# nghiant03/spine-vision

Measured on NVIDIA B200. Metric: series/sec, higher is better.
Workload: dtype fp16

## Files before the change

spine_vision_b200/csrc/svb_convnext_kernels.cuh:

```cuda
#pragma once
#include "svb_common.cuh"

namespace svb {

constexpr float LN_EPS_BACKBONE = 1e-6f;
constexpr float LN_EPS_HEAD = 1e-5f;
constexpr int DW_KX_UNROLL = 1;

__device__ __forceinline__ float gelu_fast(float x) {
    const float u = fminf(fabsf(x), 5.65685425f);
    float r = -5.20460508e-04f;
    r = fmaf(r, u, 7.39751849e-03f);
    r = fmaf(r, u, -5.25612477e-02f);
    r = fmaf(r, u, -4.59254682e-01f);
    r = fmaf(r, u, -1.15109138e+00f);
    r *= u;
    float e;
    asm("ex2.approx.ftz.f32 %0, %1;" : "=f"(e) : "f"(r));
    const float h = (0.5f * x) * e;
    return fmaxf(x, 0.0f) - fabsf(h);
}
__device__ __forceinline__ float gelu_exact(float x) { return 0.5f * x * (1.0f + erff(x * 0.70710678118654752f)); }

constexpr int STEM_TPW = 4;
// ... 871 lines not shown
                uint32_t r[32];
                tmem_ld_32x32(tmem_base + ((uint32_t)(q * 32) << 16) + (uint32_t)(as * BN + slice * CW + c * 32), r);
                if (MODE == GEMM_RESID) {
                    if (c > 0 && lane == 0) {
                        bulk_wait_read<0>();
                        mbar_expect_tx(rf, Cfg::EPI_BUF_BYTES);
                        tma_load_2d(ebuf_p, &resid_map, rf, col, row0);
                    }
                } else {
                    if (lane == 0) bulk_wait_read<0>();
                    __syncwarp();
                }
                tmem_ld_wait();
                if (MODE == GEMM_RESID) {
                    mbar_wait(rf, rph);
                    rph ^= 1u;
                }
#pragma unroll
                for (int i = 0; i < 4; ++i) {
                    const uint32_t addr = row_off + ((((uint32_t)i) ^ swz) << 4);
                    const float4 b0 = __ldg(reinterpret_cast<const float4*>(bias + col) + 2 * i);
                    const float4 b1 = __ldg(reinterpret_cast<const float4*>(bias + col) + 2 * i + 1);
                    uint64_t v01, v23, v45, v67;
                    if (MODE == GEMM_LNGELU) {
                        const float4 s0 = __ldg(reinterpret_cast<const float4*>(gamma + col) + 2 * i);
                        const float4 s1 = __ldg(reinterpret_cast<const float4*>(gamma + col) + 2 * i + 1);
                        v01 = fma2(ra2, pk2(__uint_as_float(r[8 * i + 0]), __uint_as_float(r[8 * i + 1])), fma2(rb2, pk2(s0.x, s0.y), pk2(b0.x, b0.y)));
                        v23 = fma2(ra2, pk2(__uint_as_float(r[8 * i + 2]), __uint_as_float(r[8 * i + 3])), fma2(rb2, pk2(s0.z, s0.w), pk2(b0.z, b0.w)));
                        v45 = fma2(ra2, pk2(__uint_as_float(r[8 * i + 4]), __uint_as_float(r[8 * i + 5])), fma2(rb2, pk2(s1.x, s1.y), pk2(b1.x, b1.y)));
                        v67 = fma2(ra2, pk2(__uint_as_float(r[8 * i + 6]), __uint_as_float(r[8 * i + 7])), fma2(rb2, pk2(s1.z, s1.w), pk2(b1.z, b1.w)));
                    } else {
                        v01 = add2(pk2(__uint_as_float(r[8 * i + 0]), __uint_as_float(r[8 * i + 1])), pk2(b0.x, b0.y));
                        v23 = add2(pk2(__uint_as_float(r[8 * i + 2]), __uint_as_float(r[8 * i + 3])), pk2(b0.z, b0.w));
                        v45 = add2(pk2(__uint_as_float(r[8 * i + 4]), __uint_as_float(r[8 * i + 5])), pk2(b1.x, b1.y));
                        v67 = add2(pk2(__uint_as_float(r[8 * i + 6]), __uint_as_float(r[8 * i + 7])), pk2(b1.z, b1.w));
                    }
                    uint4 o;
                    if (MODE == GEMM_GELU || MODE == GEMM_LNGELU) {
                        o = make_uint4(gelu_pack2<T>(v01), gelu_pack2<T>(v23), gelu_pack2<T>(v45), gelu_pack2<T>(v67));
                    } else {
                        if (MODE == GEMM_RESID) {
                            const float4 g0 = __ldg(reinterpret_cast<const float4*>(gamma + col) + 2 * i);
                            const float4 g1 = __ldg(reinterpret_cast<const float4*>(gamma + col) + 2 * i + 1);
                            const uint4 rv = lds128(addr);
                            const float2 x01 = Cvt<T>::unpack2(rv.x), x23 = Cvt<T>::unpack2(rv.y);
                            const float2 x45 = Cvt<T>::unpack2(rv.z), x67 = Cvt<T>::unpack2(rv.w);
                            v01 = fma2(pk2(g0.x, g0.y), v01, pk2(x01.x, x01.y));
                            v23 = fma2(pk2(g0.z, g0.w), v23, pk2(x23.x, x23.y));
                            v45 = fma2(pk2(g1.x, g1.y), v45, pk2(x45.x, x45.y));
                            v67 = fma2(pk2(g1.z, g1.w), v67, pk2(x67.x, x67.y));
                        }
                        float f0, f1, f2, f3, f4, f5, f6, f7;
                        upk2(v01, f0, f1); upk2(v23, f2, f3); upk2(v45, f4, f5); upk2(v67, f6, f7);
                        o = make_uint4(Cvt<T>::pack2(f0, f1), Cvt<T>::pack2(f2, f3), Cvt<T>::pack2(f4, f5), Cvt<T>::pack2(f6, f7));
                    }
                    sts128(addr, o);
                }
                fence_proxy_async();
                __syncwarp();
                if (lane == 0) {
                    tma_store_2d(&out_map, ebuf_p, col, row0);
                    bulk_commit();
                }
            }
            tc_fence_before();
            __syncwarp();
            if (lane == 0) {
                if (CG == 1 || rank == 0) mbar_arrive_relaxed(&tempty[as]);
                else mbar_arrive_cluster_relaxed(mapa_shared(smem_u32(&tempty[as]), 0));
            }
            if (++as == 2) { as = 0; aphase ^= 1; }
        }
        if (lane == 0) bulk_wait_all();
    }
    tc_fence_before();
    if (CG == 2) cluster_sync_all(); else __syncthreads();
    if (warp == 1) tmem_dealloc<CG>(tmem_base, Cfg::TMEM_COLS);
}

template <int C>
struct MlpCfg {
    static constexpr int HC = 64;
    static constexpr int NJ = 4 * C / HC;
    static constexpr int NB = (512 - C) / HC;
    static constexpr int KB_A = C / 64;
    static constexpr int A_BYTES = KB_A * 16384;
    static constexpr int H_BYTES = 16384;
    static constexpr int W1_KB_BYTES = 32 * 128;
    static constexpr int SLOT = KB_A * W1_KB_BYTES;
    static constexpr int W_SLOTS = C == 128 ? 7 : 5;
    static constexpr int VEC_BYTES = (4 * C + 4 * C + C + C) * 4;
    static constexpr int EPI_WARPS = 16;
    static constexpr int CH = C / 4 / 32;
    static constexpr bool STAGE_IN_H = C == 256;
    static constexpr int STAGE_BYTES = STAGE_IN_H ? 0 : EPI_WARPS * CH * 2048;
    static constexpr int NUM_THREADS = 64 + 32 * EPI_WARPS;
    static constexpr int NUM_BARS = 2 * W_SLOTS + 2 + 6 * NB + 4 + EPI_WARPS;
    static constexpr int SMEM_BYTES = A_BYTES + NB * H_BYTES + STAGE_BYTES + W_SLOTS * SLOT + VEC_BYTES + NUM_BARS * 8 + 64 + 1024;
    static constexpr int TMEM_COLS = 512;
    static_assert(C == 128 || C == 256, "Y (C columns) + NB 64-column hidden accumulators must fit 512 TMEM columns");
    static_assert(C + NB * HC <= 512, "TMEM budget");
    static_assert(SLOT == (C / 2) * 128, "W1 and W2 chunk halves are the same size");
    static_assert(!STAGE_IN_H || NB * H_BYTES >= EPI_WARPS * CH * 2048, "staging must fit the hidden buffers");
    static_assert(SMEM_BYTES <= 227 * 1024, "shared memory budget");
};

template <typename T, int C, bool LNF>
__global__ void __launch_bounds__(MlpCfg<C>::NUM_THREADS, 1)
mlp_fused_kernel(const __grid_constant__ CUtensorMap a_map, const __grid_constant__ CUtensorMap w1_map,
                 const __grid_constant__ CUtensorMap w2_map, const __grid_constant__ CUtensorMap x_map,
                 const float* __restrict__ b1, const float* __restrict__ b2, const float* __restrict__ gamma, int M,
                 const float* __restrict__ s1, const float2* __restrict__ rowstat, int stat_parts) {
    using Cfg = MlpCfg<C>;
    constexpr int NJ = Cfg::NJ, S = Cfg::W_SLOTS, NB = Cfg::NB, CH = Cfg::CH;
    extern __shared__ uint8_t smem_raw[];
    uint8_t* smem = smem_raw + ((1024u - (smem_u32(smem_raw) & 1023u)) & 1023u);
    uint8_t* sA = smem;
    uint8_t* sH = sA + Cfg::A_BYTES;
    uint8_t* sStage = sH + NB * Cfg::H_BYTES;
    uint8_t* sW = sStage + Cfg::STAGE_BYTES;
    float* sB1 = reinterpret_cast<float*>(sW + S * Cfg::SLOT);
    float* sS1 = sB1 + 4 * C;
    float* sB2 = sS1 + 4 * C;
    float* sGm = sB2 + C;
    uint64_t* bars = reinterpret_cast<uint64_t*>(reinterpret_cast<uint8_t*>(sB1) + Cfg::VEC_BYTES);
    uint64_t* wfull = bars;
    uint64_t* wempty = wfull + S;
    uint64_t* afull = wempty + S;
    uint64_t* aempty = afull + 1;
    uint64_t* hacc_full = aempty + 1;
    uint64_t* hacc_free_l = hacc_full + NB;
    uint64_t* hacc_free_p = hacc_free_l + NB;
    uint64_t* hs_full_l = hacc_free_p + NB;
    uint64_t* hs_full_p = hs_full_l + NB;
    uint64_t* hs_free = hs_full_p + NB;
    uint64_t* yfull = hs_free + NB;
    uint64_t* yfree_l = yfull + 1;
    uint64_t* yfree_p = yfree_l + 1;
    uint64_t* rfull = yfree_p + 2;
    uint32_t* tmem_ptr = reinterpret_cast<uint32_t*>(rfull + Cfg::EPI_WARPS);

    const int warp = __shfl_sync(0xffffffffu, (int)(threadIdx.x >> 5), 0), lane = threadIdx.x & 31;
    const uint32_t rank = cluster_ctarank();
    const int num_tiles = (M + 255) / 256;
    const int tile0 = (int)blockIdx.x / 2, tile_step = (int)gridDim.x / 2;

    if (warp == 0 && lane == 0) {
        tma_prefetch_desc(&a_map);
        tma_prefetch_desc(&w1_map);
        tma_prefetch_desc(&w2_map);
        tma_prefetch_desc(&x_map);
        for (int s = 0; s < S; ++s) { mbar_init(&wfull[s], 1); mbar_init(&wempty[s], 1); }
        mbar_init(afull, 1);
        mbar_init(aempty, 1);
        for (int s = 0; s < NB; ++s) {
            mbar_init(&hacc_full[s], 1);
            mbar_init(&hacc_free_l[s], Cfg::EPI_WARPS);
            mbar_init(&hacc_free_p[s], 1);
            mbar_init(&hs_full_l[s], Cfg::EPI_WARPS);
            mbar_init(&hs_full_p[s], 1);
            mbar_init(&hs_free[s], 1);
        }
        mbar_init(yfull, 1);
        mbar_init(yfree_l, Cfg::EPI_WARPS);
        mbar_init(yfree_p, 1);
        for (int s = 0; s < Cfg::EPI_WARPS; ++s) mbar_init(&rfull[s], 1);
        mbar_fence_init();
    }
    if (warp == 1) tmem_alloc<2>(tmem_ptr, Cfg::TMEM_COLS);
    for (int i = threadIdx.x; i < 4 * C; i += Cfg::NUM_THREADS) {
        sB1[i] = __ldg(b1 + i);
        sS1[i] = LNF ? __ldg(s1 + i) : 0.f;
    }
    for (int i = threadIdx.x; i < C; i += Cfg::NUM_THREADS) {
        sB2[i] = __ldg(b2 + i);
        sGm[i] = __ldg(gamma + i);
    }
    tc_fence_before();
    cluster_sync_all();
    tc_fence_after();
    const uint32_t tmem_base = *tmem_ptr;
    const uint32_t tm_y = tmem_base, tm_h = tmem_base + (uint32_t)C;
    pdl_launch_dependents();

    if (warp == 0) {
        if (lane == 0) {
            pdl_wait();
            int slot = 0;
            uint32_t wphase = 0, tcount = 0;
            auto next_slot = [&]() -> uint8_t* {
                mbar_wait(&wempty[slot], wphase ^ 1);
                if (rank == 0) mbar_expect_tx(&wfull[slot], 2 * Cfg::SLOT);
                return sW + slot * Cfg::SLOT;
            };
            auto advance = [&]() { if (++slot == S) { slot = 0; wphase ^= 1; } };
            auto load_w1 = [&](int j) {
                uint8_t* dst = next_slot();
                const uint32_t lb = mapa_shared(smem_u32(&wfull[slot]), 0);
#pragma unroll
                for (int kb = 0; kb < Cfg::KB_A; ++kb)
                    tma_load_2d_pair(dst + kb * Cfg::W1_KB_BYTES, &w1_map, lb, kb * 64, j * 64 + (int)rank * 32);
                advance();
            };
            auto load_w2 = [&](int jj) {
                uint8_t* dst = next_slot();
                const uint32_t lb = mapa_shared(smem_u32(&wfull[slot]), 0);
                tma_load_2d_pair(dst, &w2_map, lb, jj * 64, (int)rank * (C / 2));
                advance();
            };
            for (int tile = tile0; tile < num_tiles; tile += tile_step, ++tcount) {
                const int row_a = (tile * 2 + (int)rank) * 128;
                mbar_wait(aempty, (tcount & 1) ^ 1);
                if (rank == 0) mbar_expect_tx(afull, 2 * Cfg::A_BYTES);
                const uint32_t la = mapa_shared(smem_u32(afull), 0);
#pragma unroll
                for (int kb = 0; kb < Cfg::KB_A; ++kb) tma_load_2d_pair(sA + kb * 16384, &a_map, la, kb * 64, row_a);
                for (int j = 0; j < NJ + NB - 1; ++j) {
                    if (j < NJ) load_w1(j);
                    if (j >= NB - 1) load_w2(j - (NB - 1));
                }
            }
        }
    } else if (warp == 1) {
        if (rank == 0) {
            const uint32_t lead = elect_one() ? 1u : 0u;
            constexpr uint32_t idesc1 = (1u << 4) | (UmmaFmt<T>::v << 7) | (UmmaFmt<T>::v << 10) | ((uint32_t)(Cfg::HC >> 3) << 17) |
                                        ((uint32_t)(256 >> 4) << 24);
            constexpr uint32_t idesc2 = (1u << 4) | (UmmaFmt<T>::v << 7) | (UmmaFmt<T>::v << 10) | ((uint32_t)(C >> 3) << 17) |
                                        ((uint32_t)(256 >> 4) << 24);
            int slot = 0;
            uint32_t wphase = 0, tcount = 0, j1 = 0, j2 = 0;
            auto wait_slot = [&]() -> uint32_t {
                mbar_wait(&wfull[slot], wphase);
                tc_fence_after();
                return smem_u32(sW + slot * Cfg::SLOT);
            };
            auto release_slot = [&]() {
                tc_commit_if<2>(lead, &wempty[slot]);
                if (++slot == S) { slot = 0; wphase ^= 1; }
            };
            for (int tile = tile0; tile < num_tiles; tile += tile_step, ++tcount) {
                mbar_wait(afull, tcount & 1);
                tc_fence_after();
                for (int j = 0; j < NJ + NB - 1; ++j) {
                    if (j < NJ) {
                        const uint32_t hb = j1 % NB, par = ((j1 / NB) & 1) ^ 1;
                        mbar_wait(&hacc_free_l[hb], par);
                        mbar_wait(&hacc_free_p[hb], par);
                        tc_fence_after();
                        const uint32_t d = tm_h + hb * Cfg::HC;
                        {
                            const uint32_t wb = wait_slot();
#pragma unroll
                            for (int kb = 0; kb < Cfg::KB_A; ++kb) {
                                const uint64_t adesc = make_sw128_kmajor_desc(smem_u32(sA + kb * 16384));
                                const uint64_t bdesc = make_sw128_kmajor_desc(wb + kb * Cfg::W1_KB_BYTES);
#pragma unroll
                                for (int k = 0; k < 4; ++k)
                                    tc_mma_f16_if<2>(lead, d, adesc + 2 * k, bdesc + 2 * k, idesc1, (kb | k) != 0 ? 1u : 0u);
                            }
                            release_slot();
                        }
                        if (j == NJ - 1) tc_commit_if<2>(lead, aempty);
                        tc_commit_if<2>(lead, &hacc_full[hb]);
                        ++j1;
                    }
                    if (j >= NB - 1) {
                        const int jj = j - (NB - 1);
                        const uint32_t hb = j2 % NB, par = (j2 / NB) & 1;
                        mbar_wait(&hs_full_l[hb], par);
                        mbar_wait(&hs_full_p[hb], par);
                        if (jj == 0) {
                            mbar_wait(yfree_l, (tcount & 1) ^ 1);
                            mbar_wait(yfree_p, (tcount & 1) ^ 1);
                        }
                        tc_fence_after();
                        const uint32_t hs = smem_u32(sH + hb * Cfg::H_BYTES);
                        {
                            const uint32_t wb = wait_slot();
                            const uint64_t adesc = make_sw128_kmajor_desc(hs);
                            const uint64_t bdesc = make_sw128_kmajor_desc(wb);
#pragma unroll
                            for (int k = 0; k < 4; ++k)
                                tc_mma_f16_if<2>(lead, tm_y, adesc + 2 * k, bdesc + 2 * k, idesc2, (jj > 0 || k > 0) ? 1u : 0u);
                            release_slot();
                        }
                        tc_commit_if<2>(lead, &hs_free[hb]);
                        ++j2;
                    }
                }
                tc_commit_if<2>(lead, yfull);
            }
        } else if (lane == 0 && rank == 1) {
            uint32_t j1 = 0, tcount = 0;
            for (int tile = tile0; tile < num_tiles; tile += tile_step, ++tcount) {
                for (int j = 0; j < NJ; ++j, ++j1) {
                    const uint32_t hb = j1 % NB, par = (j1 / NB) & 1;
                    mbar_wait(&hacc_free_l[hb], par);
                    mbar_arrive_cluster_relaxed(mapa_shared(smem_u32(&hacc_free_p[hb]), 0));
                    mbar_wait(&hs_full_l[hb], par);
                    mbar_arrive_cluster_relaxed(mapa_shared(smem_u32(&hs_full_p[hb]), 0));
                }
                mbar_wait(yfree_l, tcount & 1);
                mbar_arrive_cluster_relaxed(mapa_shared(smem_u32(yfree_p), 0));
            }
        }
    } else {
        const int ew = warp - 2;
        const int q = warp & 3;
        const int slice = ew >> 2;
        const int r = q * 32 + lane;
        const uint32_t lane_sel = (uint32_t)(q * 32) << 16;
        uint32_t j1 = 0, tcount = 0, rph = 0;
        uint8_t* stage_p = (Cfg::STAGE_IN_H ? sH : sStage) + ew * CH * 2048;
        const uint32_t stage_a = smem_u32(stage_p);
        constexpr int CW = C / 4;
        pdl_wait();
        for (int tile = tile0; tile < num_tiles; tile += tile_step, ++tcount) {
            const int row0 = (tile * 2 + (int)rank) * 128 + q * 32;
            uint64_t ra2 = 0, rb2 = 0;
            if (LNF) {
                float2 rs = make_float2(0.f, 0.f);
                if (row0 + lane < M) {
                    if (stat_parts == 0) {
                        rs = __ldg(rowstat + row0 + lane);
                    } else {
                        const float2* rp = rowstat + (size_t)(row0 + lane) * (size_t)stat_parts;
                        float sm = 0.f, sq = 0.f;
                        for (int p = 0; p < stat_parts; ++p) { const float2 v = __ldg(rp + p); sm += v.x; sq += v.y; }
                        const float mu = sm * (1.0f / (float)C);
                        const float var = fmaxf(fmaf(-mu, mu, sq * (1.0f / (float)C)), 0.0f);
                        const float rstd = 1.0f / sqrtf(var + LN_EPS_BACKBONE);
                        rs = make_float2(rstd, -mu * rstd);
                    }
                }
                ra2 = pk2(rs.x, rs.x);
                rb2 = pk2(rs.y, rs.y);
            }
            if (!Cfg::STAGE_IN_H && row0 < M && lane == 0) {
                mbar_expect_tx(&rfull[ew], CH * 2048);
#pragma unroll
                for (int c = 0; c < CH; ++c) tma_load_2d(stage_p + c * 2048, &x_map, &rfull[ew], slice * CW + c * 32, row0);
            }
            constexpr bool PF = C == 256;
            float vbuf[2][16];
            if (PF) {
                const uint32_t hb = j1 % NB, u = (j1 / NB) & 1;
                mbar_wait(&hacc_full[hb], u);
                tc_fence_after();
                TmemLd<16>::ld(tm_h + lane_sel + hb * Cfg::HC + (uint32_t)(slice * 16), vbuf[0]);
            }
#pragma unroll PF ? NJ : 1
            for (int j = 0; j < NJ; ++j, ++j1) {
                const uint32_t hb = j1 % NB, u = (j1 / NB) & 1;
                const int hcol = j * Cfg::HC + slice * 16;
                float (&v)[16] = vbuf[PF ? (j & 1) : 0];
                if (!PF) {
                    mbar_wait(&hacc_full[hb], u);
                    tc_fence_after();
                    TmemLd<16>::ld(tm_h + lane_sel + hb * Cfg::HC + (uint32_t)(slice * 16), v);
                }
                tmem_ld_wait();
                tc_fence_before();
                __syncwarp();
                if (lane == 0) mbar_arrive_relaxed(&hacc_free_l[hb]);
                if (PF && j + 1 < NJ) {
                    const uint32_t hn = (j1 + 1) % NB, un = ((j1 + 1) / NB) & 1;
                    mbar_wait(&hacc_full[hn], un);
                    tc_fence_after();
                    TmemLd<16>::ld(tm_h + lane_sel + hn * Cfg::HC + (uint32_t)(slice * 16), vbuf[(j + 1) & 1]);
                }
                float4 bias[4], sn[4];
#pragma unroll
                for (int i = 0; i < 4; ++i) {
                    bias[i] = reinterpret_cast<const float4*>(sB1 + hcol)[i];
                    if (LNF) sn[i] = reinterpret_cast<const float4*>(sS1 + hcol)[i];
                }
                mbar_wait(&hs_free[hb], u ^ 1);
                const uint32_t dst = smem_u32(sH + hb * Cfg::H_BYTES) + (uint32_t)(r * 128);
#pragma unroll
                for (int i = 0; i < 2; ++i) {
                    const float4 c0 = bias[2 * i], c1 = bias[2 * i + 1];
                    uint64_t v01, v23, v45, v67;
                    if (LNF) {
                        const float4 s0 = sn[2 * i], s1v = sn[2 * i + 1];
                        v01 = fma2(ra2, pk2(v[8 * i + 0], v[8 * i + 1]), fma2(rb2, pk2(s0.x, s0.y), pk2(c0.x, c0.y)));
                        v23 = fma2(ra2, pk2(v[8 * i + 2], v[8 * i + 3]), fma2(rb2, pk2(s0.z, s0.w), pk2(c0.z, c0.w)));
                        v45 = fma2(ra2, pk2(v[8 * i + 4], v[8 * i + 5]), fma2(rb2, pk2(s1v.x, s1v.y), pk2(c1.x, c1.y)));
                        v67 = fma2(ra2, pk2(v[8 * i + 6], v[8 * i + 7]), fma2(rb2, pk2(s1v.z, s1v.w), pk2(c1.z, c1.w)));
                    } else {
                        v01 = add2(pk2(v[8 * i + 0], v[8 * i + 1]), pk2(c0.x, c0.y));
                        v23 = add2(pk2(v[8 * i + 2], v[8 * i + 3]), pk2(c0.z, c0.w));
                        v45 = add2(pk2(v[8 * i + 4], v[8 * i + 5]), pk2(c1.x, c1.y));
                        v67 = add2(pk2(v[8 * i + 6], v[8 * i + 7]), pk2(c1.z, c1.w));
                    }
                    const uint32_t piece = (uint32_t)(slice * 2 + i);
                    sts128(dst + ((piece ^ ((uint32_t)r & 7u)) << 4),
                           make_uint4(gelu_pack2<T>(v01), gelu_pack2<T>(v23), gelu_pack2<T>(v45), gelu_pack2<T>(v67)));
                }
                fence_proxy_async();
                __syncwarp();
                if (lane == 0) mbar_arrive_relaxed(&hs_full_l[hb]);
            }
            const uint32_t swz = ((uint32_t)lane >> 1) & 3u;
            mbar_wait(yfull, tcount & 1);
            tc_fence_after();
            if (Cfg::STAGE_IN_H && row0 < M && lane == 0) {
                mbar_expect_tx(&rfull[ew], CH * 2048);
#pragma unroll
                for (int c = 0; c < CH; ++c) tma_load_2d(stage_p + c * 2048, &x_map, &rfull[ew], slice * CW + c * 32, row0);
            }
            if (row0 < M) {
                mbar_wait(&rfull[ew], rph);
                rph ^= 1u;
            }
#pragma unroll
            for (int c = 0; c < CH; ++c) {
                const int col = slice * CW + c * 32;
                uint32_t v[32];
                tmem_ld_32x32(tm_y + lane_sel + (uint32_t)col, v);
                tmem_ld_wait();
                if (c == CH - 1) {
                    tc_fence_before();
                    __syncwarp();
                    if (lane == 0) mbar_arrive_relaxed(yfree_l);
                }
                if (row0 < M) {
                    const uint32_t row_off = stage_a + (uint32_t)(c * 2048) + (uint32_t)lane * 64u;
#pragma unroll
                    for (int i = 0; i < 4; ++i) {
                        const uint32_t addr = row_off + ((((uint32_t)i) ^ swz) << 4);
                        const float4 c0 = reinterpret_cast<const float4*>(sB2 + col)[2 * i];
                        const float4 c1 = reinterpret_cast<const float4*>(sB2 + col)[2 * i + 1];
                        const float4 g0 = reinterpret_cast<const float4*>(sGm + col)[2 * i];
                        const float4 g1 = reinterpret_cast<const float4*>(sGm + col)[2 * i + 1];
                        const uint4 rv = lds128(addr);
                        const float2 x01 = Cvt<T>::unpack2(rv.x), x23 = Cvt<T>::unpack2(rv.y);
                        const float2 x45 = Cvt<T>::unpack2(rv.z), x67 = Cvt<T>::unpack2(rv.w);
                        const uint64_t v01 = fma2(pk2(g0.x, g0.y), add2(pk2(__uint_as_float(v[8 * i + 0]), __uint_as_float(v[8 * i + 1])), pk2(c0.x, c0.y)), pk2(x01.x, x01.y));
                        const uint64_t v23 = fma2(pk2(g0.z, g0.w), add2(pk2(__uint_as_float(v[8 * i + 2]), __uint_as_float(v[8 * i + 3])), pk2(c0.z, c0.w)), pk2(x23.x, x23.y));
                        const uint64_t v45 = fma2(pk2(g1.x, g1.y), add2(pk2(__uint_as_float(v[8 * i + 4]), __uint_as_float(v[8 * i + 5])), pk2(c1.x, c1.y)), pk2(x45.x, x45.y));
                        const uint64_t v67 = fma2(pk2(g1.z, g1.w), add2(pk2(__uint_as_float(v[8 * i + 6]), __uint_as_float(v[8 * i + 7])), pk2(c1.z, c1.w)), pk2(x67.x, x67.y));
                        float f0, f1, f2, f3, f4, f5, f6, f7;
                        upk2(v01, f0, f1); upk2(v23, f2, f3); upk2(v45, f4, f5); upk2(v67, f6, f7);
                        sts128(addr, make_uint4(Cvt<T>::pack2(f0, f1), Cvt<T>::pack2(f2, f3), Cvt<T>::pack2(f4, f5), Cvt<T>::pack2(f6, f7)));
                    }
                }
            }
            if (row0 < M) {
                fence_proxy_async();
                __syncwarp();
                if (lane == 0) {
#pragma unroll
                    for (int c = 0; c < CH; ++c) tma_store_2d(&x_map, stage_p + c * 2048, slice * CW + c * 32, row0);
                    bulk_commit();
                }
            }
            if (lane == 0) bulk_wait_read<0>();
            if (Cfg::STAGE_IN_H) asm volatile("bar.sync 1, %0;" ::"n"(Cfg::EPI_WARPS * 32) : "memory");
            else __syncwarp();
        }
        if (lane == 0) bulk_wait_all();
    }
    tc_fence_before();
    cluster_sync_all();
    if (warp == 1) tmem_dealloc<2>(tmem_base, Cfg::TMEM_COLS);
}

struct DwTc2Cfg {
    static constexpr int CC = 64, NB = 112;
    static constexpr int B_BYTES = NB * 128;
    static constexpr int B_TOTAL = 7 * B_BYTES;
    static constexpr int A_STAGE = (256 + 6 * 32) * 128;
    static constexpr int A_STAGES = 2;
    static constexpr int STAT_BYTES = 2 * 3 * 128 * 8;
    static constexpr int EPI_WARPS = 16;
    static constexpr int NUM_THREADS = 64 + 32 * EPI_WARPS;
    static constexpr int SMEM_BYTES = B_TOTAL + A_STAGES * A_STAGE + STAT_BYTES + 256 + 1024;
    static constexpr int TMEM_COLS = 512;
    static_assert(B_BYTES % 1024 == 0 && A_STAGE % 1024 == 0, "swizzle atoms");
    static_assert(SMEM_BYTES <= 227 * 1024, "shared memory budget");
};

template <int DELTA>
__device__ __forceinline__ void shfl_add(float& acc, float v, float mask, int width) {
    if (DELTA == 0) acc += v;
    else if (DELTA > 0) acc = fmaf(__shfl_down_sync(0xffffffffu, v, DELTA, width), mask, acc);
    else acc = fmaf(__shfl_up_sync(0xffffffffu, v, -DELTA, width), mask, acc);
}

template <int DELTA>
__device__ __forceinline__ void shfl_add_h2(float& a0, float& a1, float v0, float v1, uint32_t mask_h2, int width) {
    uint32_t h;
    asm("cvt.rn.satfinite.f16x2.f32 %0, %1, %2;" : "=r"(h) : "f"(v1), "f"(v0));
    const uint32_t t = DELTA > 0 ? __shfl_down_sync(0xffffffffu, h, DELTA, width) : __shfl_up_sync(0xffffffffu, h, -DELTA, width);
    asm("{\n\t.reg .f16 tl, th, ml, mh;\n\tmov.b32 {tl, th}, %2;\n\tmov.b32 {ml, mh}, %3;\n\t"
        "fma.rn.f32.f16 %0, tl, ml, %0;\n\tfma.rn.f32.f16 %1, th, mh, %1;\n\t}\n"
        : "+f"(a0), "+f"(a1)
        : "r"(t), "r"(mask_h2));
}
__device__ __forceinline__ void stg256(void* p, const uint32_t (&o)[8]) {
    asm volatile("st.global.v8.b32 [%0], {%1, %2, %3, %4, %5, %6, %7, %8};" ::"l"(p), "r"(o[0]), "r"(o[1]), "r"(o[2]), "r"(o[3]), "r"(o[4]),
                 "r"(o[5]), "r"(o[6]), "r"(o[7])
                 : "memory");
}

template <typename T, int CG>
__global__ void __launch_bounds__(DwTc2Cfg::NUM_THREADS, 1)
dwconv_rawtc_kernel(const __grid_constant__ CUtensorMap x_map, const __grid_constant__ CUtensorMap b_map,
                    const float* __restrict__ bdw, T* __restrict__ out, float2* __restrict__ stat_part, int C, int H, int W,
                    int rowpx ,
                    int nwin , int units_y, int num_units, int b0) {
    using Cfg = DwTc2Cfg;
    extern __shared__ uint8_t smem_raw[];
    uint8_t* smem = smem_raw + ((1024u - (smem_u32(smem_raw) & 1023u)) & 1023u);
    uint8_t* sB = smem;
    uint8_t* sA = smem + Cfg::B_TOTAL;
    float2* sStat = reinterpret_cast<float2*>(sA + Cfg::A_STAGES * Cfg::A_STAGE);
    uint64_t* bars = reinterpret_cast<uint64_t*>(reinterpret_cast<uint8_t*>(sStat) + Cfg::STAT_BYTES);
    uint64_t* bfull = bars;
    uint64_t* afull = bars + 1;
    uint64_t* aempty = afull + 2;
    uint64_t* tfull = aempty + 2;
    uint64_t* tempty = tfull + 4;
    uint64_t* sfull = tempty + 4;
    uint32_t* tmem_ptr = reinterpret_cast<uint32_t*>(sfull + 2);

    const int warp = __shfl_sync(0xffffffffu, (int)(threadIdx.x >> 5), 0), lane = threadIdx.x & 31;
    const int NCH = C / Cfg::CC;
    const uint32_t rank = CG == 2 ? cluster_ctarank() : 0u;
    const int unit_id = (int)blockIdx.x / CG;
    const int k = unit_id % NCH;
    const int u0 = unit_id / NCH, ustep = ((int)gridDim.x / CG) / NCH;
    constexpr int B_CTA = Cfg::B_BYTES / CG;
    const bool mode_b = nwin > 1 || rowpx != W;
    const int rows_unit = mode_b ? 8 : 256 / W;
    const int units_img = nwin * units_y;
    const uint32_t a_bytes = (uint32_t)(256 + 6 * rowpx) * 128u;

    if (threadIdx.x == 0) {
        tma_prefetch_desc(&x_map);
        tma_prefetch_desc(&b_map);
        mbar_init(bfull, 1);
        for (int s = 0; s < 2; ++s) { mbar_init(&afull[s], 1); mbar_init(&aempty[s], 1); mbar_init(&sfull[s], 12); }
        for (int s = 0; s < 4; ++s) { mbar_init(&tfull[s], 1); mbar_init(&tempty[s], 4 * CG); }
// ... 714 lines not shown
```

Measured before the change: 4384.

## Split MLP epilogue into dedicated residual warps with double-buffered Y accumulator

Result: no change. 4396 (median of 6 runs) (+0.3%).

```diff
diff --git a/spine_vision_b200/csrc/svb_convnext_kernels.cuh b/spine_vision_b200/csrc/svb_convnext_kernels.cuh
--- a/spine_vision_b200/csrc/svb_convnext_kernels.cuh
+++ b/spine_vision_b200/csrc/svb_convnext_kernels.cuh
@@ -977,26 +977,28 @@
 struct MlpCfg {
     static constexpr int HC = 64;
     static constexpr int NJ = 4 * C / HC;
-    static constexpr int NB = (512 - C) / HC;
+    static constexpr int YB = C == 128 ? 2 : 1;
+    static constexpr int NB = (512 - YB * C) / HC;
     static constexpr int KB_A = C / 64;
     static constexpr int A_BYTES = KB_A * 16384;
     static constexpr int H_BYTES = 16384;
     static constexpr int W1_KB_BYTES = 32 * 128;
     static constexpr int SLOT = KB_A * W1_KB_BYTES;
-    static constexpr int W_SLOTS = C == 128 ? 7 : 5;
+    static constexpr int W_SLOTS = C == 128 ? 7 : 4;
     static constexpr int VEC_BYTES = (4 * C + 4 * C + C + C) * 4;
-    static constexpr int EPI_WARPS = 16;
-    static constexpr int CH = C / 4 / 32;
-    static constexpr bool STAGE_IN_H = C == 256;
-    static constexpr int STAGE_BYTES = STAGE_IN_H ? 0 : EPI_WARPS * CH * 2048;
-    static constexpr int NUM_THREADS = 64 + 32 * EPI_WARPS;
-    static constexpr int NUM_BARS = 2 * W_SLOTS + 2 + 6 * NB + 4 + EPI_WARPS;
+    static constexpr int GELU_WARPS = 16;
+    static constexpr int RES_WARPS = 4;
+    static constexpr int CB = C / 32;
+    static constexpr int RB = C == 128 ? CB : 2;
+    static constexpr int STAGE_BYTES = RES_WARPS * RB * 2048;
+    static constexpr int NUM_THREADS = 32 * (2 + RES_WARPS + GELU_WARPS);
+    static constexpr int NUM_BARS = 2 * W_SLOTS + 2 + 6 * NB + 2 * YB + RES_WARPS * RB;
     static constexpr int SMEM_BYTES = A_BYTES + NB * H_BYTES + STAGE_BYTES + W_SLOTS * SLOT + VEC_BYTES + NUM_BARS * 8 + 64 + 1024;
     static constexpr int TMEM_COLS = 512;
     static_assert(C == 128 || C == 256, "Y (C columns) + NB 64-column hidden accumulators must fit 512 TMEM columns");
-    static_assert(C + NB * HC <= 512, "TMEM budget");
+    static_assert(YB * C + NB * HC <= 512, "TMEM budget");
     static_assert(SLOT == (C / 2) * 128, "W1 and W2 chunk halves are the same size");
-    static_assert(!STAGE_IN_H || NB * H_BYTES >= EPI_WARPS * CH * 2048, "staging must fit the hidden buffers");
+    static_assert(RB >= 2 && RB <= CB, "residual box ring");
     static_assert(SMEM_BYTES <= 227 * 1024, "shared memory budget");
 };
 
@@ -1007,7 +1009,7 @@
                  const float* __restrict__ b1, const float* __restrict__ b2, const float* __restrict__ gamma, int M,
                  const float* __restrict__ s1, const float2* __restrict__ rowstat, int stat_parts) {
     using Cfg = MlpCfg<C>;
-    constexpr int NJ = Cfg::NJ, S = Cfg::W_SLOTS, NB = Cfg::NB, CH = Cfg::CH;
+    constexpr int NJ = Cfg::NJ, S = Cfg::W_SLOTS, NB = Cfg::NB, YB = Cfg::YB, CB = Cfg::CB, RB = Cfg::RB;
     extern __shared__ uint8_t smem_raw[];
     uint8_t* smem = smem_raw + ((1024u - (smem_u32(smem_raw) & 1023u)) & 1023u);
     uint8_t* sA = smem;
@@ -1030,10 +1032,9 @@
     uint64_t* hs_full_p = hs_full_l + NB;
     uint64_t* hs_free = hs_full_p + NB;
     uint64_t* yfull = hs_free + NB;
-    uint64_t* yfree_l = yfull + 1;
-    uint64_t* yfree_p = yfree_l + 1;
-    uint64_t* rfull = yfree_p + 2;
-    uint32_t* tmem_ptr = reinterpret_cast<uint32_t*>(rfull + Cfg::EPI_WARPS);
+    uint64_t* yfree = yfull + YB;
+    uint64_t* rfull = yfree + YB;
+    uint32_t* tmem_ptr = reinterpret_cast<uint32_t*>(rfull + Cfg::RES_WARPS * RB);
 
     const int warp = __shfl_sync(0xffffffffu, (int)(threadIdx.x >> 5), 0), lane = threadIdx.x & 31;
     const uint32_t rank = cluster_ctarank();
@@ -1050,16 +1051,17 @@
         mbar_init(aempty, 1);
         for (int s = 0; s < NB; ++s) {
             mbar_init(&hacc_full[s], 1);
-            mbar_init(&hacc_free_l[s], Cfg::EPI_WARPS);
+            mbar_init(&hacc_free_l[s], Cfg::GELU_WARPS);
             mbar_init(&hacc_free_p[s], 1);
-            mbar_init(&hs_full_l[s], Cfg::EPI_WARPS);
+            mbar_init(&hs_full_l[s], Cfg::GELU_WARPS);
             mbar_init(&hs_full_p[s], 1);
             mbar_init(&hs_free[s], 1);
         }
-        mbar_init(yfull, 1);
-        mbar_init(yfree_l, Cfg::EPI_WARPS);
-        mbar_init(yfree_p, 1);
-        for (int s = 0; s < Cfg::EPI_WARPS; ++s) mbar_init(&rfull[s], 1);
+        for (int s = 0; s < YB; ++s) {
+            mbar_init(&yfull[s], 1);
+            mbar_init(&yfree[s], 2 * Cfg::RES_WARPS);
+        }
+        for (int s = 0; s < Cfg::RES_WARPS * RB; ++s) mbar_init(&rfull[s], 1);
         mbar_fence_init();
     }
     if (warp == 1) tmem_alloc<2>(tmem_ptr, Cfg::TMEM_COLS);
@@ -1075,253 +1077,177 @@
     cluster_sync_all();
     tc_fence_after();
     const uint32_t tmem_base = *tmem_ptr;
-    const uint32_t tm_y = tmem_base, tm_h = tmem_base + (uint32_t)C;
+    const uint32_t tm_y = tmem_base, tm_h = tmem_base + (uint32_t)(YB * C);
     pdl_launch_dependents();
 
-    if (warp == 0) {
-        if (lane == 0) {
-            pdl_wait();
-            int slot = 0;
-            uint32_t wphase = 0, tcount = 0;
-            auto next_slot = [&]() -> uint8_t* {
-                mbar_wait(&wempty[slot], wphase ^ 1);
-                if (rank == 0) mbar_expect_tx(&wfull[slot], 2 * Cfg::SLOT);
-                return sW + slot * Cfg::SLOT;
-            };
-            auto advance = [&]() { if (++slot == S) { slot = 0; wphase ^= 1; } };
-            auto load_w1 = [&](int j) {
-                uint8_t* dst = next_slot();
-                const uint32_t lb = mapa_shared(smem_u32(&wfull[slot]), 0);
-#pragma unroll
-                for (int kb = 0; kb < Cfg::KB_A; ++kb)
-                    tma_load_2d_pair(dst + kb * Cfg::W1_KB_BYTES, &w1_map, lb, kb * 64, j * 64 + (int)rank * 32);
-                advance();
-            };
-            auto load_w2 = [&](int jj) {
-                uint8_t* dst = next_slot();
-                const uint32_t lb = mapa_shared(smem_u32(&wfull[slot]), 0);
-                tma_load_2d_pair(dst, &w2_map, lb, jj * 64, (int)rank * (C / 2));
-                advance();
-            };
-            for (int tile = tile0; tile < num_tiles; tile += tile_step, ++tcount) {
-                const int row_a = (tile * 2 + (int)rank) * 128;
-                mbar_wait(aempty, (tcount & 1) ^ 1);
-                if (rank == 0) mbar_expect_tx(afull, 2 * Cfg::A_BYTES);
-                const uint32_t la = mapa_shared(smem_u32(afull), 0);
-#pragma unroll
-                for (int kb = 0; kb < Cfg::KB_A; ++kb) tma_load_2d_pair(sA + kb * 16384, &a_map, la, kb * 64, row_a);
-                for (int j = 0; j < NJ + NB - 1; ++j) {
-                    if (j < NJ) load_w1(j);
-                    if (j >= NB - 1) load_w2(j - (NB - 1));
-                }
-            }
-        }
-    } else if (warp == 1) {
-        if (rank == 0) {
-            const uint32_t lead = elect_one() ? 1u : 0u;
-            constexpr uint32_t idesc1 = (1u << 4) | (UmmaFmt<T>::v << 7) | (UmmaFmt<T>::v << 10) | ((uint32_t)(Cfg::HC >> 3) << 17) |
-                                        ((uint32_t)(256 >> 4) << 24);
-            constexpr uint32_t idesc2 = (1u << 4) | (UmmaFmt<T>::v << 7) | (UmmaFmt<T>::v << 10) | ((uint32_t)(C >> 3) << 17) |
-                                        ((uint32_t)(256 >> 4) << 24);
-            int slot = 0;
-            uint32_t wphase = 0, tcount = 0, j1 = 0, j2 = 0;
-            auto wait_slot = [&]() -> uint32_t {
-                mbar_wait(&wfull[slot], wphase);
-                tc_fence_after();
-                return smem_u32(sW + slot * Cfg::SLOT);
-            };
-            auto release_slot = [&]() {
-                tc_commit_if<2>(lead, &wempty[slot]);
-                if (++slot == S) { slot = 0; wphase ^= 1; }
-            };
-            for (int tile = tile0; tile < num_tiles; tile += tile_step, ++tcount) {
-                mbar_wait(afull, tcount & 1);
-                tc_fence_after();
-                for (int j = 0; j < NJ + NB - 1; ++j) {
-                    if (j < NJ) {
-                        const uint32_t hb = j1 % NB, par = ((j1 / NB) & 1) ^ 1;
+    if (warp < 2) {
+        if (warp == 0) {
+            if (lane == 0) {
+                pdl_wait();
+                int slot = 0;
+                uint32_t wphase = 0, tcount = 0;
+                auto next_slot = [&]() -> uint8_t* {
+                    mbar_wait(&wempty[slot], wphase ^ 1);
+                    if (rank == 0) mbar_expect_tx(&wfull[slot], 2 * Cfg::SLOT);
+                    return sW + slot * Cfg::SLOT;
+                };
+                auto advance = [&]() { if (++slot == S) { slot = 0; wphase ^= 1; } };
+                auto load_w1 = [&](int j) {
+                    uint8_t* dst = next_slot();
+                    const uint32_t lb = mapa_shared(smem_u32(&wfull[slot]), 0);
+#pragma unroll
+                    for (int kb = 0; kb < Cfg::KB_A; ++kb)
+                        tma_load_2d_pair(dst + kb * Cfg::W1_KB_BYTES, &w1_map, lb, kb * 64, j * 64 + (int)rank * 32);
+                    advance();
+                };
+                auto load_w2 = [&](int jj) {
+                    uint8_t* dst = next_slot();
+                    const uint32_t lb = mapa_shared(smem_u32(&wfull[slot]), 0);
+                    tma_load_2d_pair(dst, &w2_map, lb, jj * 64, (int)rank * (C / 2));
+                    advance();
+                };
+                for (int tile = tile0; tile < num_tiles; tile += tile_step, ++tcount) {
+                    const int row_a = (tile * 2 + (int)rank) * 128;
+                    mbar_wait(aempty, (tcount & 1) ^ 1);
+                    if (rank == 0) mbar_expect_tx(afull, 2 * Cfg::A_BYTES);
+                    const uint32_t la = mapa_shared(smem_u32(afull), 0);
+#pragma unroll
+                    for (int kb = 0; kb < Cfg::KB_A; ++kb) tma_load_2d_pair(sA + kb * 16384, &a_map, la, kb * 64, row_a);
+                    for (int j = 0; j < NJ + NB - 1; ++j) {
+                        if (j < NJ) load_w1(j);
+                        if (j >= NB - 1) load_w2(j - (NB - 1));
+                    }
+                }
+            }
+        } else if (warp == 1) {
+            if (rank == 0) {
+                const uint32_t lead = elect_one() ? 1u : 0u;
+                constexpr uint32_t idesc1 = (1u << 4) | (UmmaFmt<T>::v << 7) | (UmmaFmt<T>::v << 10) | ((uint32_t)(Cfg::HC >> 3) << 17) |
+                                            ((uint32_t)(256 >> 4) << 24);
+                constexpr uint32_t idesc2 = (1u << 4) | (UmmaFmt<T>::v << 7) | (UmmaFmt<T>::v << 10) | ((uint32_t)(C >> 3) << 17) |
+                                            ((uint32_t)(256 >> 4) << 24);
+                int slot = 0;
+                uint32_t wphase = 0, tcount = 0, j1 = 0, j2 = 0;
+                auto wait_slot = [&]() -> uint32_t {
+                    mbar_wait(&wfull[slot], wphase);
+                    tc_fence_after();
+                    return smem_u32(sW + slot * Cfg::SLOT);
+                };
+                auto release_slot = [&]() {
+                    tc_commit_if<2>(lead, &wempty[slot]);
+                    if (++slot == S) { slot = 0; wphase ^= 1; }
+                };
+                for (int tile = tile0; tile < num_tiles; tile += tile_step, ++tcount) {
+                    const uint32_t yb = tcount % YB, yu = (tcount / YB) & 1, tm_yb = tm_y + yb * (uint32_t)C;
+                    mbar_wait(afull, tcount & 1);
+                    tc_fence_after();
+                    for (int j = 0; j < NJ + NB - 1; ++j) {
+                        if (j < NJ) {
+                            const uint32_t hb = j1 % NB, par = ((j1 / NB) & 1) ^ 1;
+                            mbar_wait(&hacc_free_l[hb], par);
+                            mbar_wait(&hacc_free_p[hb], par);
+                            tc_fence_after();
+                            const uint32_t d = tm_h + hb * Cfg::HC;
+                            {
+                                const uint32_t wb = wait_slot();
+#pragma unroll
+                                for (int kb = 0; kb < Cfg::KB_A; ++kb) {
+                                    const uint64_t adesc = make_sw128_kmajor_desc(smem_u32(sA + kb * 16384));
+                                    const uint64_t bdesc = make_sw128_kmajor_desc(wb + kb * Cfg::W1_KB_BYTES);
+#pragma unroll
+                                    for (int k = 0; k < 4; ++k)
+                                        tc_mma_f16_if<2>(lead, d, adesc + 2 * k, bdesc + 2 * k, idesc1, (kb | k) != 0 ? 1u : 0u);
+                                }
+                                release_slot();
+                            }
+                            if (j == NJ - 1) tc_commit_if<2>(lead, aempty);
+                            tc_commit_if<2>(lead, &hacc_full[hb]);
+                            ++j1;
+                        }
+                        if (j >= NB - 1) {
+                            const int jj = j - (NB - 1);
+                            const uint32_t hb = j2 % NB, par = (j2 / NB) & 1;
+                            mbar_wait(&hs_full_l[hb], par);
+                            mbar_wait(&hs_full_p[hb], par);
+                            if (jj == 0) {
+                                mbar_wait(&yfree[yb], yu ^ 1);
+                            }
+                            tc_fence_after();
+                            const uint32_t hs = smem_u32(sH + hb * Cfg::H_BYTES);
+                            {
+                                const uint32_t wb = wait_slot();
+                                const uint64_t adesc = make_sw128_kmajor_desc(hs);
+                                const uint64_t bdesc = make_sw128_kmajor_desc(wb);
+#pragma unroll
+                                for (int k = 0; k < 4; ++k)
+                                    tc_mma_f16_if<2>(lead, tm_yb, adesc + 2 * k, bdesc + 2 * k, idesc2, (jj > 0 || k > 0) ? 1u : 0u);
+                                release_slot();
+                            }
+                            tc_commit_if<2>(lead, &hs_free[hb]);
+                            ++j2;
+                        }
+                    }
+                    tc_commit_if<2>(lead, &yfull[yb]);
+                }
+            } else if (lane == 0 && rank == 1) {
+                uint32_t j1 = 0, tcount = 0;
+                for (int tile = tile0; tile < num_tiles; tile += tile_step, ++tcount) {
+                    for (int j = 0; j < NJ; ++j, ++j1) {
+                        const uint32_t hb = j1 % NB, par = (j1 / NB) & 1;
                         mbar_wait(&hacc_free_l[hb], par);
-                        mbar_wait(&hacc_free_p[hb], par);
-                        tc_fence_after();
-                        const uint32_t d = tm_h + hb * Cfg::HC;
-                        {
-                            const uint32_t wb = wait_slot();
-#pragma unroll
-                            for (int kb = 0; kb < Cfg::KB_A; ++kb) {
-                                const uint64_t adesc = make_sw128_kmajor_desc(smem_u32(sA + kb * 16384));
-                                const uint64_t bdesc = make_sw128_kmajor_desc(wb + kb * Cfg::W1_KB_BYTES);
-#pragma unroll
-                                for (int k = 0; k < 4; ++k)
-                                    tc_mma_f16_if<2>(lead, d, adesc + 2 * k, bdesc + 2 * k, idesc1, (kb | k) != 0 ? 1u : 0u);
-                            }
-                            release_slot();
-                        }
-                        if (j == NJ - 1) tc_commit_if<2>(lead, aempty);
-                        tc_commit_if<2>(lead, &hacc_full[hb]);
-                        ++j1;
-                    }
-                    if (j >= NB - 1) {
-                        const int jj = j - (NB - 1);
-                        const uint32_t hb = j2 % NB, par = (j2 / NB) & 1;
+                        mbar_arrive_cluster_relaxed(mapa_shared(smem_u32(&hacc_free_p[hb]), 0));
                         mbar_wait(&hs_full_l[hb], par);
-                        mbar_wait(&hs_full_p[hb], par);
-                        if (jj == 0) {
-                            mbar_wait(yfree_l, (tcount & 1) ^ 1);
-                            mbar_wait(yfree_p, (tcount & 1) ^ 1);
-                        }
-                        tc_fence_after();
-                        const uint32_t hs = smem_u32(sH + hb * Cfg::H_BYTES);
-                        {
-                            const uint32_t wb = wait_slot();
-                            const uint64_t adesc = make_sw128_kmajor_desc(hs);
-                            const uint64_t bdesc = make_sw128_kmajor_desc(wb);
-#pragma unroll
-                            for (int k = 0; k < 4; ++k)
-                                tc_mma_f16_if<2>(lead, tm_y, adesc + 2 * k, bdesc + 2 * k, idesc2, (jj > 0 || k > 0) ? 1u : 0u);
-                            release_slot();
-                        }
-                        tc_commit_if<2>(lead, &hs_free[hb]);
-                        ++j2;
-                    }
-                }
-                tc_commit_if<2>(lead, yfull);
-            }
-        } else if (lane == 0 && rank == 1) {
-            uint32_t j1 = 0, tcount = 0;
-            for (int tile = tile0; tile < num_tiles; tile += tile_step, ++tcount) {
-                for (int j = 0; j < NJ; ++j, ++j1) {
-                    const uint32_t hb = j1 % NB, par = (j1 / NB) & 1;
-                    mbar_wait(&hacc_free_l[hb], par);
-                    mbar_arrive_cluster_relaxed(mapa_shared(smem_u32(&hacc_free_p[hb]), 0));
-                    mbar_wait(&hs_full_l[hb], par);
-                    mbar_arrive_cluster_relaxed(mapa_shared(smem_u32(&hs_full_p[hb]), 0));
-                }
-                mbar_wait(yfree_l, tcount & 1);
-                mbar_arrive_cluster_relaxed(mapa_shared(smem_u32(yfree_p), 0));
-            }
-        }
-    } else {
-        const int ew = warp - 2;
+                        mbar_arrive_cluster_relaxed(mapa_shared(smem_u32(&hs_full_p[hb]), 0));
+                    }
+                }
+            }
+        }
+    } else if (warp < 2 + Cfg::RES_WARPS) {
         const int q = warp & 3;
-        const int slice = ew >> 2;
-        const int r = q * 32 + lane;
         const uint32_t lane_sel = (uint32_t)(q * 32) << 16;
-        uint32_t j1 = 0, tcount = 0, rph = 0;
-        uint8_t* stage_p = (Cfg::STAGE_IN_H ? sH : sStage) + ew * CH * 2048;
-        const uint32_t stage_a = smem_u32(stage_p);
-        constexpr int CW = C / 4;
+        const uint32_t swz = ((uint32_t)lane >> 1) & 3u;
+        uint8_t* ring = sStage + q * RB * 2048;
+        uint64_t* rf = rfull + q * RB;
+        const int nbox = tile0 < num_tiles ? ((num_tiles - 1 - tile0) / tile_step + 1) * CB : 0;
+        auto box_row = [&](int b) { return ((tile0 + (b / CB) * tile_step) * 2 + (int)rank) * 128 + q * 32; };
+        auto load_box = [&](int b) {
+            if (b < nbox && box_row(b) < M) {
+                const int s = b % RB;
+                mbar_expect_tx(&rf[s], 2048);
+                tma_load_2d(ring + s * 2048, &x_map, &rf[s], (b % CB) * 32, box_row(b));
+            }
+        };
         pdl_wait();
-        for (int tile = tile0; tile < num_tiles; tile += tile_step, ++tcount) {
-            const int row0 = (tile * 2 + (int)rank) * 128 + q * 32;
-            uint64_t ra2 = 0, rb2 = 0;
-            if (LNF) {
-                float2 rs = make_float2(0.f, 0.f);
-                if (row0 + lane < M) {
-                    if (stat_parts == 0) {
-                        rs = __ldg(rowstat + row0 + lane);
-                    } else {
-                        const float2* rp = rowstat + (size_t)(row0 + lane) * (size_t)stat_parts;
-                        float sm = 0.f, sq = 0.f;
-                        for (int p = 0; p < stat_parts; ++p) { const float2 v = __ldg(rp + p); sm += v.x; sq += v.y; }
-                        const float mu = sm * (1.0f / (float)C);
-                        const float var = fmaxf(fmaf(-mu, mu, sq * (1.0f / (float)C)), 0.0f);
-                        const float rstd = 1.0f / sqrtf(var + LN_EPS_BACKBONE);
-                        rs = make_float2(rstd, -mu * rstd);
-                    }
-                }
-                ra2 = pk2(rs.x, rs.x);
-                rb2 = pk2(rs.y, rs.y);
-            }
-            if (!Cfg::STAGE_IN_H && row0 < M && lane == 0) {
-                mbar_expect_tx(&rfull[ew], CH * 2048);
-#pragma unroll
-                for (int c = 0; c < CH; ++c) tma_load_2d(stage_p + c * 2048, &x_map, &rfull[ew], slice * CW + c * 32, row0);
-            }
-            constexpr bool PF = C == 256;
-            float vbuf[2][16];
-            if (PF) {
-                const uint32_t hb = j1 % NB, u = (j1 / NB) & 1;
-                mbar_wait(&hacc_full[hb], u);
-                tc_fence_after();
-                TmemLd<16>::ld(tm_h + lane_sel + hb * Cfg::HC + (uint32_t)(slice * 16), vbuf[0]);
-            }
-#pragma unroll PF ? NJ : 1
-            for (int j = 0; j < NJ; ++j, ++j1) {
-                const uint32_t hb = j1 % NB, u = (j1 / NB) & 1;
-                const int hcol = j * Cfg::HC + slice * 16;
-                float (&v)[16] = vbuf[PF ? (j & 1) : 0];
-                if (!PF) {
-                    mbar_wait(&hacc_full[hb], u);
-                    tc_fence_after();
-                    TmemLd<16>::ld(tm_h + lane_sel + hb * Cfg::HC + (uint32_t)(slice * 16), v);
-                }
+        if (lane == 0)
+            for (int b = 0; b < RB - 1; ++b) load_box(b);
+        uint32_t tcount = 0;
+        for (int b = 0; b < nbox; ++tcount) {
+            const uint32_t yb = tcount % YB;
+            const int row0 = box_row(b);
+            mbar_wait(&yfull[yb], (tcount / YB) & 1);
+            tc_fence_after();
+#pragma unroll 1
+            for (int c = 0; c < CB; ++c, ++b) {
+                const int col = c * 32, s = b % RB;
+                if (lane == 0) {
+                    bulk_wait_read<0>();
+                    load_box(b + RB - 1);
+                }
+                __syncwarp();
+                uint32_t v[32];
+                tmem_ld_32x32(tm_y + yb * (uint32_t)C + lane_sel + (uint32_t)col, v);
                 tmem_ld_wait();
-                tc_fence_before();
-                __syncwarp();
-                if (lane == 0) mbar_arrive_relaxed(&hacc_free_l[hb]);
-                if (PF && j + 1 < NJ) {
-                    const uint32_t hn = (j1 + 1) % NB, un = ((j1 + 1) / NB) & 1;
-                    mbar_wait(&hacc_full[hn], un);
-                    tc_fence_after();
-                    TmemLd<16>::ld(tm_h + lane_sel + hn * Cfg::HC + (uint32_t)(slice * 16), vbuf[(j + 1) & 1]);
-                }
-                float4 bias[4], sn[4];
-#pragma unroll
-                for (int i = 0; i < 4; ++i) {
-                    bias[i] = reinterpret_cast<const float4*>(sB1 + hcol)[i];
-                    if (LNF) sn[i] = reinterpret_cast<const float4*>(sS1 + hcol)[i];
-                }
-                mbar_wait(&hs_free[hb], u ^ 1);
-                const uint32_t dst = smem_u32(sH + hb * Cfg::H_BYTES) + (uint32_t)(r * 128);
-#pragma unroll
-                for (int i = 0; i < 2; ++i) {
-                    const float4 c0 = bias[2 * i], c1 = bias[2 * i + 1];
-                    uint64_t v01, v23, v45, v67;
-                    if (LNF) {
-                        const float4 s0 = sn[2 * i], s1v = sn[2 * i + 1];
-                        v01 = fma2(ra2, pk2(v[8 * i + 0], v[8 * i + 1]), fma2(rb2, pk2(s0.x, s0.y), pk2(c0.x, c0.y)));
-                        v23 = fma2(ra2, pk2(v[8 * i + 2], v[8 * i + 3]), fma2(rb2, pk2(s0.z, s0.w), pk2(c0.z, c0.w)));
-                        v45 = fma2(ra2, pk2(v[8 * i + 4], v[8 * i + 5]), fma2(rb2, pk2(s1v.x, s1v.y), pk2(c1.x, c1.y)));
-                        v67 = fma2(ra2, pk2(v[8 * i + 6], v[8 * i + 7]), fma2(rb2, pk2(s1v.z, s1v.w), pk2(c1.z, c1.w)));
-                    } else {
-                        v01 = add2(pk2(v[8 * i + 0], v[8 * i + 1]), pk2(c0.x, c0.y));
-                        v23 = add2(pk2(v[8 * i + 2], v[8 * i + 3]), pk2(c0.z, c0.w));
-                        v45 = add2(pk2(v[8 * i + 4], v[8 * i + 5]), pk2(c1.x, c1.y));
-                        v67 = add2(pk2(v[8 * i + 6], v[8 * i + 7]), pk2(c1.z, c1.w));
-                    }
-                    const uint32_t piece = (uint32_t)(slice * 2 + i);
-                    sts128(dst + ((piece ^ ((uint32_t)r & 7u)) << 4),
-                           make_uint4(gelu_pack2<T>(v01), gelu_pack2<T>(v23), gelu_pack2<T>(v45), gelu_pack2<T>(v67)));
-                }
-                fence_proxy_async();
-                __syncwarp();
-                if (lane == 0) mbar_arrive_relaxed(&hs_full_l[hb]);
-            }
-            const uint32_t swz = ((uint32_t)lane >> 1) & 3u;
-            mbar_wait(yfull, tcount & 1);
-            tc_fence_after();
-            if (Cfg::STAGE_IN_H && row0 < M && lane == 0) {
-                mbar_expect_tx(&rfull[ew], CH * 2048);
-#pragma unroll
-                for (int c = 0; c < CH; ++c) tma_load_2d(stage_p + c * 2048, &x_map, &rfull[ew], slice * CW + c * 32, row0);
-            }
-            if (row0 < M) {
-                mbar_wait(&rfull[ew], rph);
-                rph ^= 1u;
-            }
-#pragma unroll
-            for (int c = 0; c < CH; ++c) {
-                const int col = slice * CW + c * 32;
-                uint32_t v[32];
-                tmem_ld_32x32(tm_y + lane_sel + (uint32_t)col, v);
-                tmem_ld_wait();
-                if (c == CH - 1) {
+                if (c == CB - 1) {
                     tc_fence_before();
                     __syncwarp();
-                    if (lane == 0) mbar_arrive_relaxed(yfree_l);
+                    if (lane == 0) {
+                        if (rank == 0) mbar_arrive_relaxed(&yfree[yb]);
+                        else mbar_arrive_cluster_relaxed(mapa_shared(smem_u32(&yfree[yb]), 0));
+                    }
                 }
                 if (row0 < M) {
-                    const uint32_t row_off = stage_a + (uint32_t)(c * 2048) + (uint32_t)lane * 64u;
+                    mbar_wait(&rf[s], (uint32_t)(b / RB) & 1u);
+                    const uint32_t row_off = smem_u32(ring + s * 2048) + (uint32_t)lane * 64u;
 #pragma unroll
                     for (int i = 0; i < 4; ++i) {
                         const uint32_t addr = row_off + ((((uint32_t)i) ^ swz) << 4);
@@ -1340,22 +1266,100 @@
                         upk2(v01, f0, f1); upk2(v23, f2, f3); upk2(v45, f4, f5); upk2(v67, f6, f7);
                         sts128(addr, make_uint4(Cvt<T>::pack2(f0, f1), Cvt<T>::pack2(f2, f3), Cvt<T>::pack2(f4, f5), Cvt<T>::pack2(f6, f7)));
                     }
-                }
-            }
-            if (row0 < M) {
+                    fence_proxy_async();
+                    __syncwarp();
+                    if (lane == 0) {
+                        tma_store_2d(&x_map, ring + s * 2048, col, row0);
+                        bulk_commit();
+                    }
+                }
+            }
+        }
+        if (lane == 0) bulk_wait_all();
+    } else {
+        const int gw = warp - 2 - Cfg::RES_WARPS;
+        const int q = warp & 3;
+        const int slice = gw >> 2;
+        const int r = q * 32 + lane;
+        const uint32_t lane_sel = (uint32_t)(q * 32) << 16;
+        uint32_t j1 = 0;
+        pdl_wait();
+        for (int tile = tile0; tile < num_tiles; tile += tile_step) {
+            const int row0 = (tile * 2 + (int)rank) * 128 + q * 32;
+            uint64_t ra2 = 0, rb2 = 0;
+            if (LNF) {
+                float2 rs = make_float2(0.f, 0.f);
+                if (row0 + lane < M) {
+                    if (stat_parts == 0) {
+                        rs = __ldg(rowstat + row0 + lane);
+                    } else {
+                        const float2* rp = rowstat + (size_t)(row0 + lane) * (size_t)stat_parts;
+                        float sm = 0.f, sq = 0.f;
+                        for (int p = 0; p < stat_parts; ++p) { const float2 v = __ldg(rp + p); sm += v.x; sq += v.y; }
+                        const float mu = sm * (1.0f / (float)C);
+                        const float var = fmaxf(fmaf(-mu, mu, sq * (1.0f / (float)C)), 0.0f);
+                        const float rstd = 1.0f / sqrtf(var + LN_EPS_BACKBONE);
+                        rs = make_float2(rstd, -mu * rstd);
+                    }
+                }
+                ra2 = pk2(rs.x, rs.x);
+                rb2 = pk2(rs.y, rs.y);
+            }
+            constexpr bool PF = C == 256;
+            float vbuf[2][16];
+            if (PF) {
+                const uint32_t hb = j1 % NB, u = (j1 / NB) & 1;
+                mbar_wait(&hacc_full[hb], u);
+                tc_fence_after();
+                TmemLd<16>::ld(tm_h + lane_sel + hb * Cfg::HC + (uint32_t)(slice * 16), vbuf[0]);
+            }
+#pragma unroll PF ? NJ : 1
+            for (int j = 0; j < NJ; ++j, ++j1) {
+                const uint32_t hb = j1 % NB, u = (j1 / NB) & 1;
+                const int hcol = j * Cfg::HC + slice * 16;
+                float (&v)[16] = vbuf[PF ? (j & 1) : 0];
+                if (!PF) {
+                    mbar_wait(&hacc_full[hb], u);
+                    tc_fence_after();
+                    TmemLd<16>::ld(tm_h + lane_sel + hb * Cfg::HC + (uint32_t)(slice * 16), v);
+                }
+                tmem_ld_wait();
+                tc_fence_before();
+                __syncwarp();
+                if (lane == 0) mbar_arrive_relaxed(&hacc_free_l[hb]);
+                if (PF && j + 1 < NJ) {
+                    const uint32_t hn = (j1 + 1) % NB, un = ((j1 + 1) / NB) & 1;
+                    mbar_wait(&hacc_full[hn], un);
+                    tc_fence_after();
+                    TmemLd<16>::ld(tm_h + lane_sel + hn * Cfg::HC + (uint32_t)(slice * 16), vbuf[(j + 1) & 1]);
+                }
+                mbar_wait(&hs_free[hb], u ^ 1);
+                const uint32_t dst = smem_u32(sH + hb * Cfg::H_BYTES) + (uint32_t)(r * 128);
+#pragma unroll
+                for (int i = 0; i < 2; ++i) {
+                    const float4 c0 = reinterpret_cast<const float4*>(sB1 + hcol)[2 * i], c1 = reinterpret_cast<const float4*>(sB1 + hcol)[2 * i + 1];
+                    uint64_t v01, v23, v45, v67;
+                    if (LNF) {
+                        const float4 s0 = reinterpret_cast<const float4*>(sS1 + hcol)[2 * i], s1v = reinterpret_cast<const float4*>(sS1 + hcol)[2 * i + 1];
+                        v01 = fma2(ra2, pk2(v[8 * i + 0], v[8 * i + 1]), fma2(rb2, pk2(s0.x, s0.y), pk2(c0.x, c0.y)));
+                        v23 = fma2(ra2, pk2(v[8 * i + 2], v[8 * i + 3]), fma2(rb2, pk2(s0.z, s0.w), pk2(c0.z, c0.w)));
+                        v45 = fma2(ra2, pk2(v[8 * i + 4], v[8 * i + 5]), fma2(rb2, pk2(s1v.x, s1v.y), pk2(c1.x, c1.y)));
+                        v67 = fma2(ra2, pk2(v[8 * i + 6], v[8 * i + 7]), fma2(rb2, pk2(s1v.z, s1v.w), pk2(c1.z, c1.w)));
+                    } else {
+                        v01 = add2(pk2(v[8 * i + 0], v[8 * i + 1]), pk2(c0.x, c0.y));
+                        v23 = add2(pk2(v[8 * i + 2], v[8 * i + 3]), pk2(c0.z, c0.w));
+                        v45 = add2(pk2(v[8 * i + 4], v[8 * i + 5]), pk2(c1.x, c1.y));
+                        v67 = add2(pk2(v[8 * i + 6], v[8 * i + 7]), pk2(c1.z, c1.w));
+                    }
+                    const uint32_t piece = (uint32_t)(slice * 2 + i);
+                    sts128(dst + ((piece ^ ((uint32_t)r & 7u)) << 4),
+                           make_uint4(gelu_pack2<T>(v01), gelu_pack2<T>(v23), gelu_pack2<T>(v45), gelu_pack2<T>(v67)));
+                }
                 fence_proxy_async();
                 __syncwarp();
-                if (lane == 0) {
-#pragma unroll
-                    for (int c = 0; c < CH; ++c) tma_store_2d(&x_map, stage_p + c * 2048, slice * CW + c * 32, row0);
-                    bulk_commit();
-                }
-            }
-            if (lane == 0) bulk_wait_read<0>();
-            if (Cfg::STAGE_IN_H) asm volatile("bar.sync 1, %0;" ::"n"(Cfg::EPI_WARPS * 32) : "memory");
-            else __syncwarp();
-        }
-        if (lane == 0) bulk_wait_all();
+                if (lane == 0) mbar_arrive_relaxed(&hs_full_l[hb]);
+            }
+        }
     }
     tc_fence_before();
     cluster_sync_all();
```
